# Apokleos/kata-xpu-device-plugin

Hardware: NVIDIA H100
Metric: pci.ids parse GB/s (x1000 text + 2^20-key join); device lookups/s reported beside it (higher is better)
Workload: dtype u8

## Files before the change

### kata-xpu-device-plugin_b200/csrc/api.cu

```cuda
#include <algorithm>
#include <cstdlib>
#include <new>
#include <vector>

#include "internal.cuh"
#include "pciids5.cu"
#include "finalize.cuh"
#include "small.cuh"
#include "scan.cuh"

void kx_exchange_destroy(kxpu_ctx *ctx);

static const char *kx_err_names[] = {
    "ok", "invalid argument", "CUDA error", "no sm_90 GPU available", "output buffer too small",
    "table capacity exceeded", "NCCL / peer exchange unavailable or failed", "input outside the supported domain", "out of memory"};

extern "C" const char *kxpu_strerror(int32_t status) {
    int i = -status;
    if (i < 0 || i > 8) return "unknown status";
    return kx_err_names[i];
}

extern "C" const char *kxpu_last_error(kxpu_ctx *ctx) {
    if (!ctx) return "null ctx";
    static thread_local char copy[sizeof(ctx->err)];
    std::lock_guard<std::mutex> g(ctx->mu);
    memcpy(copy, ctx->err, sizeof copy);
    copy[sizeof copy - 1] = 0;
    return copy;
}
extern "C" uint64_t kxpu_launch_count(kxpu_ctx *ctx) { return ctx ? ctx->launches : 0; }

int32_t kx_ctx_create_on(int32_t ordinal, kxpu_ctx **out) {
    if (!out) return KXPU_E_INVALID;
    *out = nullptr;
    int count = 0;
    if (cudaGetDeviceCount(&count) != cudaSuccess || count <= 0 || ordinal < 0 || ordinal >= count) {
        cudaGetLastError();
        return KXPU_E_NOGPU;
    }
    cudaDeviceProp prop;
    if (cudaGetDeviceProperties(&prop, ordinal) != cudaSuccess) return KXPU_E_NOGPU;
    if (prop.major != 9 || prop.minor != 0) return KXPU_E_NOGPU;
    kxpu_ctx *c = new (std::nothrow) kxpu_ctx();
    if (!c) return KXPU_E_NOMEM;
    c->device = ordinal;
    c->sm_count = prop.multiProcessorCount;
    if (cudaSetDevice(ordinal) != cudaSuccess || cudaStreamCreateWithFlags(&c->stream, cudaStreamNonBlocking) != cudaSuccess) {
        delete c;
        return KXPU_E_CUDA;
    }
    bool ok = true;
    for (int i = 0; i < 2 * KXPU_T_COUNT; i++) ok = ok && cudaEventCreate(&c->ev[i]) == cudaSuccess;
    ok = ok && cudaEventCreate(&c->ev_user[0]) == cudaSuccess && cudaEventCreate(&c->ev_user[1]) == cudaSuccess;
    ok = ok && cudaMallocHost((void **)&c->h_ctl, (KX_C_COUNT + 64) * sizeof(uint32_t)) == cudaSuccess;
    if (!ok) {
        cudaGetLastError();
        kxpu_ctx_destroy(c);
        return KXPU_E_CUDA;
    }
    cudaMemPool_t pool;
    if (cudaDeviceGetDefaultMemPool(&pool, ordinal) == cudaSuccess) {
        uint64_t thr = ~0ull;
        cudaMemPoolSetAttribute(pool, cudaMemPoolAttrReleaseThreshold, &thr);
    }
    cudaFuncSetAttribute(kxparse5::parse_kernel_v5, cudaFuncAttributeMaxDynamicSharedMemorySize,
                         (int)(sizeof(kxparse5::WarpSmem5) * kxparse::WARPS));
    const char *fr = getenv("KXPU_RCH");
    c->force_rch = (fr && fr[0] >= '1' && fr[0] <= '8' && !fr[1]) ? fr[0] - '0' : 0;
    c->no_small = getenv("KXPU_NO_SMALL") != nullptr;
    c->no_zero_copy = getenv("KXPU_NO_ZERO_COPY") != nullptr;
    if (const char *sw = getenv("KXPU_SCAN_W")) { const int v = atoi(sw); c->force_scan_w = (v == 8 || v == 16 || v == 32) ? v : 0; }
    if (const char *el = getenv("KXPU_SCAN_EPOCH_LIMIT")) {
        char *end = nullptr;
        const unsigned long long v = (el[0] >= '0' && el[0] <= '9') ? strtoull(el, &end, 10) : 0;
        if (end && !*end && v >= 2 && v <= (1ull << 24)) c->scan_epoch_limit = (uint32_t)v;
    }
    *out = c;
    return KXPU_OK;
}

extern "C" int32_t kxpu_ctx_create(int32_t ordinal, kxpu_ctx **out) { return kx_ctx_create_on(ordinal, out); }

extern "C" int32_t kxpu_ctx_destroy(kxpu_ctx *ctx) {
    if (!ctx) return KXPU_E_INVALID;
// ... 181 lines not shown
            break;
        }
    }
    if (!found) {
        KxArena a;
        a.cap = cap; a.blob_cap = blob_cap; a.range_bytes = need_range;
        a.bytes = arena_layout(cap, blob_cap, need_range).total;
        cudaError_t e = cudaMalloc(&a.p, a.bytes);
        if (e != cudaSuccess) {
            cudaGetLastError();
            for (KxArena &p : ctx->pool) cudaFree(p.p);
            ctx->pool.clear();
            e = cudaMalloc(&a.p, a.bytes);
        }
        if (e != cudaSuccess) {
            cudaGetLastError();
            KX_SET_ERR(ctx, "cudaMalloc(%zu) for a table arena -> %s", a.bytes, cudaGetErrorString(e));
            delete t;
            return e == cudaErrorMemoryAllocation ? KXPU_E_NOMEM : KXPU_E_CUDA;
        }
        arena_reset(ctx, a);
        t->arena = a;
    }
    const ArenaLayout L = arena_layout(cap, blob_cap, t->arena.range_bytes);
    uint8_t *b = (uint8_t *)t->arena.p;
    t->cap = cap;
    uint32_t lg = 0;
    while ((1u << lg) < cap) lg++;
    t->shift = 32 - lg;
    t->dev.slots = (KxSlot *)(b + L.o_slots);
    t->dev.vendor_first = (unsigned long long *)(b + L.o_vfirst);
    t->dev.trunc = (unsigned long long *)(b + L.o_trunc);
    t->dev.counters = (uint32_t *)(b + L.o_counters);
    t->dev.cap = cap;
    t->dev.shift = t->shift;
    t->dev.max_keys = cap / 2;
    t->range_words = (unsigned long long *)(b + L.o_range);
    t->row_key = (uint32_t *)(b + L.o_row_key);
    t->row_line = (unsigned long long *)(b + L.o_row_line);
    t->row_anchor = (unsigned long long *)(b + L.o_row_anchor);
    t->row_name_off = (uint32_t *)(b + L.o_row_noff);
    t->row_name_len = (uint32_t *)(b + L.o_row_nlen);
    t->sel = (uint32_t *)(b + L.o_sel);
    t->blob = b + L.o_blob;
    t->blob_cap = blob_cap;
    t->rows_cap = cap + 1;
    *out = t;
    return KXPU_OK;
}

void kx_table_release(kxpu_ctx *ctx, kxpu_table *t) {
    if (!t) return;
    if (t->arena.p) {
        if (ctx->pool.size() >= 4) {
            cudaStreamSynchronize(ctx->stream);
            cudaFree(ctx->pool.front().p);
            ctx->pool.erase(ctx->pool.begin());
        }
        arena_reset(ctx, t->arena);
        ctx->pool.push_back(t->arena);
    }
    delete t;
}

uint32_t kx_initial_blob_cap(kxpu_ctx *ctx, size_t n) {
    const uint32_t by_text = (uint32_t)std::min<size_t>(std::max<size_t>(n, 256), 4u << 20);
    return ctx->blob_hint > by_text ? ctx->blob_hint : by_text;
}

bool kx_grow_cap(uint32_t *cap, bool table_full) {
    if (*cap >= (1u << 28)) return false;
    const uint32_t sh = table_full ? 4u : 2u;
    *cap = (*cap >> (28u - sh)) ? (1u << 28) : (*cap << sh);
    return true;
}

void kx_note_table_size(kxpu_ctx *ctx, uint32_t nkeys, uint32_t blob_used, uint32_t blob_cap) {
    uint32_t ideal = 1u << 16;
    while (ideal < (1u << 28) && ideal / 2 < nkeys + nkeys / 8) ideal <<= 1;
    ctx->cap_hint = ideal;
    ctx->blob_hint = blob_cap > (4u << 20) && blob_used > (2u << 20) ? blob_cap : 0u;
}

int32_t kx_launch_parse(kxpu_ctx *ctx, kxpu_table *t, const uint8_t *d_text, size_t n, unsigned long long base,
                        unsigned long long carry_in, const KxXaHook *xa) {
    using namespace kxparse;
    const uint32_t num_chunks = (uint32_t)((n + CW - 1) / CW);
    kxparse5::Params5 P;
    memset(&P, 0, sizeof P);
    if (xa) { P.xa_on = 1; P.xa_done = xa->done; P.xa = xa->p; }
    if (num_chunks == 0) {
        if (xa) {
            P.tab = t->dev;
            P.task_ctas = 0;
            kxparse5::resolve_chunks_kernel<<<kxparse5::XA_CTAS, kxparse5::RES_WARPS * 32, 0, ctx->stream>>>(P);
            KX_LAUNCHED(ctx);
            KX_CUDA(ctx, cudaGetLastError());
        }
        return KXPU_OK;
    }
    P.text = d_text; P.n = n; P.base = base; P.num_chunks = num_chunks;
    P.tma_limit = n >= (size_t)STG_BYTES ? (uint32_t)((n - STG_BYTES) / CW) + 1u : 0u;
    static int per_sm = 0;
    const size_t smem = sizeof(kxparse5::WarpSmem5) * WARPS;
    if (per_sm == 0) {
        cudaOccupancyMaxActiveBlocksPerMultiprocessor(&per_sm, kxparse5::parse_kernel_v5, NT, smem);
        if (per_sm < 1) per_sm = 1;
    }
    const uint32_t wave_warps = (uint32_t)per_sm * ctx->sm_count * WARPS;
    P.rch = std::min<uint32_t>(std::max<uint32_t>(num_chunks / (wave_warps * 8u), 1u), kxparse5::RCH5_MAX);
    if (ctx->force_rch) P.rch = (uint32_t)ctx->force_rch;
    P.num_ranges = (num_chunks + P.rch - 1) / P.rch;
    P.range_state = t->range_words;
    P.range_carry = t->range_words + P.num_ranges;
    P.lead = (uint32_t *)(t->range_words + 2 * P.num_ranges);
    P.tasks = P.lead + P.num_ranges;
    P.tab = t->dev; P.carry_in = carry_in;
    uint32_t grid = (uint32_t)per_sm * ctx->sm_count;
    const uint32_t need = (P.num_ranges + WARPS - 1) / WARPS;
    if (grid > need) grid = need;
    {
        KxTimer tm(ctx, KXPU_T_PARSE);
        kxparse5::parse_kernel_v5<<<grid, NT, smem, ctx->stream>>>(P);
        KX_LAUNCHED(ctx);
    }
    {
        KxTimer tr(ctx, KXPU_T_RESOLVE);
        kxparse5::resolve_ranges_kernel<<<(P.num_ranges + 255u) / 256u, 256, 0, ctx->stream>>>(P);
        KX_LAUNCHED(ctx);
        const uint32_t rgrid = std::min<uint32_t>(4u * ctx->sm_count, (num_chunks + kxparse5::RES_WARPS - 1) / kxparse5::RES_WARPS);
        P.task_ctas = rgrid;
        kxparse5::resolve_chunks_kernel<<<rgrid + (xa ? kxparse5::XA_CTAS : 0u), kxparse5::RES_WARPS * 32, 0, ctx->stream>>>(P);
        KX_LAUNCHED(ctx);
    }
    KX_CUDA(ctx, cudaGetLastError());
    return KXPU_OK;
}

int32_t kx_launch_trunc(kxpu_ctx *ctx, kxpu_table *t, const uint8_t *d_text, size_t n, unsigned long long base) {
    kxparse::trunc_kernel<<<1, 1024, 0, ctx->stream>>>(d_text, n, base, t->dev.trunc, t->dev.counters);
    KX_LAUNCHED(ctx);
    KX_CUDA(ctx, cudaGetLastError());
    return KXPU_OK;
}

int32_t kx_launch_finalize(kxpu_ctx *ctx, kxpu_table *t, const uint8_t *d_text, size_t n, unsigned long long base,
                           const kxx::MinView *mv, const kxx::WaitSpec *wait, const KxSlabOut *slab) {
    kxparse::FinalizeParams F;
    memset(&F, 0, sizeof F);
    if (wait) F.wait = *wait;
    F.text = d_text; F.n = n; F.base = base; F.tab = t->dev;
    if (mv) F.mv = *mv;
    else { F.mv.a = t->dev.vendor_first; F.mv.stride = 0; F.mv.n = 1; F.mv.trunc1 = t->dev.trunc; }
    F.row_key = t->row_key; F.row_line = t->row_line; F.row_anchor = t->row_anchor;
    F.row_name_off = t->row_name_off; F.row_name_len = t->row_name_len;
    F.blob = t->blob; F.blob_cap = t->blob_cap;
    if (slab) {
        F.slab_rows = reinterpret_cast<kxx::SlabRow *>(slab->rows); F.slab_rows_cap = slab->rows_cap;
        F.blob = slab->blob; F.blob_cap = slab->blob_cap;
        F.tail = slab->tail;
    }
    KxTimer tm(ctx, KXPU_T_FINALIZE);
    F.scan_w = t->cap >= (1u << 19) ? 32u : 8u;
    if (ctx->force_scan_w) F.scan_w = (uint32_t)ctx->force_scan_w;
    const unsigned batches = (t->cap + 1 + F.scan_w - 1) / F.scan_w;
    const unsigned grid = std::min<unsigned>((batches + kxparse::SF_WARPS - 1) / kxparse::SF_WARPS, 8u * ctx->sm_count);
    kxparse::select_finalize_kernel<<<grid, kxparse::SF_WARPS * 32, 0, ctx->stream>>>(F);
    KX_LAUNCHED(ctx);
    KX_CUDA(ctx, cudaGetLastError());
    return KXPU_OK;
}

int32_t kx_launch_lookup(kxpu_ctx *ctx, kxpu_table *t, const uint32_t *d_keys, size_t n, int32_t *d_rows) {
    if (n == 0) return KXPU_OK;
    KxTimer tm(ctx, KXPU_T_LOOKUP);
    size_t blocks = (n + 255) / 256;
    size_t maxb = (size_t)ctx->sm_count * 32;
    if (blocks > maxb) blocks = maxb;
    kxparse::lookup_kernel<<<(unsigned)blocks, 256, 0, ctx->stream>>>(d_keys, n, t->dev.slots, t->cap, t->shift, d_rows);
    KX_LAUNCHED(ctx);
    KX_CUDA(ctx, cudaGetLastError());
    return KXPU_OK;
}

struct KxJoin {
    const uint32_t *d_keys;
    size_t n;
    int32_t *d_rows;
    int32_t *h_rows;
    const uint8_t *src_text;
};

static void *kx_mapped_host(const void *p) {
    if (!p) return nullptr;
    cudaPointerAttributes at;
    if (cudaPointerGetAttributes(&at, p) != cudaSuccess) { cudaGetLastError(); return nullptr; }
    return at.type == cudaMemoryTypeHost ? at.devicePointer : nullptr;
}

static uint32_t small_text_chunks(kxpu_ctx *ctx) {
    if (ctx->small_chunks < 0) {
        int coop = 0, per_sm = 0;
        cudaDeviceGetAttribute(&coop, cudaDevAttrCooperativeLaunch, ctx->device);
        cudaFuncSetAttribute(kxsmall::small_load_kernel, cudaFuncAttributeMaxDynamicSharedMemorySize, kxparse::WARPS * kxparse::STG_BYTES);
        cudaOccupancyMaxActiveBlocksPerMultiprocessor(&per_sm, kxsmall::small_load_kernel, kxparse::NT, kxparse::WARPS * kxparse::STG_BYTES);
        cudaGetLastError();
        ctx->small_chunks = (coop && !ctx->no_small) ? per_sm * ctx->sm_count * kxparse::WARPS : 0;
    }
    return (uint32_t)ctx->small_chunks;
}

static int32_t launch_small(kxpu_ctx *ctx, kxpu_table *t, const uint8_t *d_text, size_t n, const KxJoin *join) {
    using namespace kxparse;
    kxsmall::SmallParams P;
    memset(&P, 0, sizeof P);
    P.text = d_text; P.n = n;
    P.num_chunks = (uint32_t)((n + CW - 1) / CW);
    P.tma_limit = n >= (size_t)STG_BYTES ? (uint32_t)((n - STG_BYTES) / CW) + 1u : 0u;
    P.state = t->range_words;
    FinalizeParams &F = P.F;
    F.text = d_text; F.n = n; F.base = 0; F.tab = t->dev;
    F.mv.a = t->dev.vendor_first; F.mv.stride = 0; F.mv.n = 1; F.mv.trunc1 = t->dev.trunc;
    F.row_key = t->row_key; F.row_line = t->row_line; F.row_anchor = t->row_anchor;
    F.row_name_off = t->row_name_off; F.row_name_len = t->row_name_len;
    F.blob = t->blob; F.blob_cap = t->blob_cap;
    if (join) { P.keys = join->d_keys; P.nq = join->n; P.rows_out = join->d_rows; }
    if (join && join->src_text) { P.text_src = join->src_text; P.h_ctl = ctx->h_ctl; }
    void *args[] = {&P};
    const unsigned grid = std::max<unsigned>((P.num_chunks + WARPS - 1) / WARPS, (unsigned)(ctx->small_chunks / WARPS));
    F.scan_w = 8u;
    while (F.scan_w < 32u && (size_t)(t->cap + 1 + F.scan_w - 1) / F.scan_w > (size_t)grid * SF_WARPS) F.scan_w *= 2u;
    if (ctx->force_scan_w) F.scan_w = (uint32_t)ctx->force_scan_w;
    static const bool trace_on = getenv("KXPU_TRACE_SMALL") != nullptr;
    long long *d_trace = nullptr;
    if (trace_on && cudaMalloc((void **)&d_trace, (size_t)grid * 128 + (size_t)P.num_chunks * 32) == cudaSuccess) { cudaMemset(d_trace, 0, (size_t)grid * 128 + (size_t)P.num_chunks * 32); P.trace = d_trace; P.F.trace = d_trace + (size_t)grid * 8 + (size_t)P.num_chunks * 4; }
    {
        KxTimer tm(ctx, KXPU_T_PARSE);
        KX_CUDA(ctx, cudaLaunchCooperativeKernel((const void *)kxsmall::small_load_kernel, dim3(grid), dim3(NT), args, (size_t)WARPS * STG_BYTES, ctx->stream));
        KX_LAUNCHED(ctx);
    }
    if (d_trace) {
        std::vector<long long> h((size_t)grid * 16 + (size_t)P.num_chunks * 4);
        cudaStreamSynchronize(ctx->stream);
        cudaMemcpy(h.data(), d_trace, h.size() * 8, cudaMemcpyDeviceToHost);
        cudaFree(d_trace);
        static const char *nm[7] = {"phase1", "barrier1", "phase2", "barrier2", "names", "barrier3", "join"};
        fprintf(stderr, "[kxpu small trace] %u CTAs, cycles min/avg/max per CTA:", grid);
        for (int k = 0; k < 7; k++) {
            long long mn = 1ll << 62, mx = 0, sum = 0, cnt = 0;
            for (unsigned b = 0; b < grid; b++) {
                if (!h[b * 8 + k + 1] || !h[b * 8 + k]) continue;
                const long long d = h[b * 8 + k + 1] - h[b * 8 + k];
                mn = std::min(mn, d); mx = std::max(mx, d); sum += d; cnt++;
            }
            if (cnt) fprintf(stderr, " %s %lld/%lld/%lld |", nm[k], mn, sum / cnt, mx);
        }
        {
            std::vector<std::pair<long long, unsigned>> v;
            for (unsigned b = 0; b < grid; b++) v.push_back({h[b * 8 + 3] - h[b * 8 + 2], b});
            std::sort(v.rbegin(), v.rend());
            fprintf(stderr, " slowest phase2 CTAs:");
            for (int k = 0; k < 6 && k < (int)v.size(); k++) fprintf(stderr, " %u:%lld", v[k].second, v[k].first);
            std::vector<std::pair<long long, unsigned>> wv;
            const long long *tw = h.data() + (size_t)grid * 8;
            for (unsigned c = 0; c < P.num_chunks; c++) wv.push_back({tw[c * 4], c});
            std::sort(wv.rbegin(), wv.rend());
            fprintf(stderr, "\n   slowest phase2 warps (chunk: cycles / before folds / entries / look-back steps):");
            for (int k = 0; k < 10 && k < (int)wv.size(); k++) {
                const unsigned c = wv[k].second;
                fprintf(stderr, " %u: %lld/%lld/%lld/%lld |", c, tw[c * 4], tw[c * 4 + 1], tw[c * 4 + 2], tw[c * 4 + 3]);
            }
            const unsigned mid = wv[wv.size() / 2].second;
            fprintf(stderr, " median %u: %lld/%lld/%lld/%lld", mid, tw[mid * 4], tw[mid * 4 + 1], tw[mid * 4 + 2], tw[mid * 4 + 3]);
            const long long *tf = h.data() + (size_t)grid * 8 + (size_t)P.num_chunks * 4;
            static const char *fn[7] = {"scan", "rounds", "sync1+claim", "sync2", "names out+rows", "long lines", "shift+sync3"};
            fprintf(stderr, "\n   names phase per CTA (thread 0), cycles min/avg/max:");
            for (int k = 0; k < 7; k++) {
                long long mn = 1ll << 62, mx = 0, sum = 0, cnt = 0;
                for (unsigned b = 0; b < grid; b++) {
                    const long long t1 = tf[b * 8 + k], t0 = k ? tf[b * 8 + k - 1] : h[b * 8 + 4];
                    if (!t1 || !t0) continue;
                    const long long d = t1 - t0;
                    mn = std::min(mn, d); mx = std::max(mx, d); sum += d; cnt++;
                }
                if (cnt) fprintf(stderr, " %s %lld/%lld/%lld |", fn[k], mn, sum / cnt, mx);
            }
        }
        fprintf(stderr, "\n");
    }
    return KXPU_OK;
}

static int32_t kx_build_table_join(kxpu_ctx *ctx, const uint8_t *d_text, size_t n, kxpu_table **out, const KxJoin *join) {
    if ((reinterpret_cast<uintptr_t>(d_text) & 15u) != 0) {
        KX_SET_ERR(ctx, "device text pointer must be 16-byte aligned");
        return KXPU_E_INVALID;
    }
    if (n >= (1ull << 44)) return KXPU_E_UNSUPPORTED;
    uint32_t cap = ctx->cap_hint;
    while (cap > (1u << 16) && (size_t)cap / 2 > n / 6 + 1) cap >>= 1;
    uint32_t blob_cap = kx_initial_blob_cap(ctx, n);
    const uint32_t num_chunks = (uint32_t)((n + kxparse::CW - 1) / kxparse::CW);
    bool have_trunc = false;
    for (int attempt = 0; attempt < 12; attempt++) {
        kxpu_table *t = nullptr;
        int32_t rc = kx_table_acquire(ctx, cap, blob_cap, num_chunks, &t);
        if (rc != KXPU_OK) return rc;
        const bool small_path = num_chunks > 0 && num_chunks <= small_text_chunks(ctx) && !have_trunc;
        if (small_path) {
            rc = launch_small(ctx, t, d_text, n, join);
        } else {
            if (join && join->src_text && attempt == 0) cudaMemcpyAsync(const_cast<uint8_t *>(d_text), join->src_text, n, cudaMemcpyDefault, ctx->stream);
            rc = kx_launch_parse(ctx, t, d_text, n, 0, 0, nullptr);
            if (rc == KXPU_OK && have_trunc) rc = kx_launch_trunc(ctx, t, d_text, n, 0);
            if (rc == KXPU_OK) rc = kx_launch_finalize(ctx, t, d_text, n, 0, nullptr, nullptr, nullptr);
            if (rc == KXPU_OK && join) rc = kx_launch_lookup(ctx, t, join->d_keys, join->n, join->d_rows);
        }
        if (rc != KXPU_OK) { kx_table_release(ctx, t); return rc; }
        const bool zero_copy = small_path && join && join->src_text;
        if (!zero_copy) {
            if (join && join->h_rows && join->n) cudaMemcpyAsync(join->h_rows, join->d_rows, join->n * 4, cudaMemcpyDeviceToHost, ctx->stream);
            cudaMemcpyAsync(ctx->h_ctl, t->dev.counters, KX_C_COUNT * 4, cudaMemcpyDeviceToHost, ctx->stream);
        }
        cudaError_t e = cudaStreamSynchronize(ctx->stream);
        if (e != cudaSuccess) {
            KX_SET_ERR(ctx, "parse/finalize failed: %s", cudaGetErrorString(e));
            kx_table_release(ctx, t);
            return KXPU_E_CUDA;
        }
        const uint32_t *h = ctx->h_ctl;
        if (h[KX_C_OVERFLOW] || h[KX_C_NKEYS] > t->dev.max_keys) {
            kx_table_release(ctx, t);
            if (!kx_grow_cap(&cap, h[KX_C_OVERFLOW] != 0)) return KXPU_E_CAPACITY;
            continue;
        }
        if (h[KX_C_NEED_TRUNC] == 2u) {
            kx_table_release(ctx, t);
            have_trunc = true;
            continue;
        }
        if (h[KX_C_BLOB_OVERFLOW]) {
            kx_table_release(ctx, t);
            if ((size_t)blob_cap >= n) return KXPU_E_CAPACITY;
            blob_cap = (uint32_t)std::min<size_t>(std::max<size_t>(n, 256), (size_t)blob_cap * 8);
            continue;
        }
        t->n_rows = h[KX_C_NSEL];
        t->blob_used = h[KX_C_BLOB_CURSOR];
        kx_note_table_size(ctx, h[KX_C_NKEYS], t->blob_used, blob_cap);
        *out = t;
        return KXPU_OK;
    }
    return KXPU_E_CAPACITY;
}

extern "C" int32_t kxpu_pciids_load_device(kxpu_ctx *ctx, const void *d_text, size_t n, kxpu_table **out) {
    KX_ENTER(ctx);
    if (!out || (!d_text && n)) return KXPU_E_INVALID;
    kx_clear_timings(ctx);
    return kx_build_table_join(ctx, (const uint8_t *)d_text, n, out, nullptr);
}

extern "C" int32_t kxpu_pciids_join_device(kxpu_ctx *ctx, const void *d_text, size_t n, const uint32_t *d_keys, size_t nq,
                                           int32_t *d_rows_out, kxpu_table **out) {
    KX_ENTER(ctx);
    if (!out || (!d_text && n) || (nq && (!d_keys || !d_rows_out))) return KXPU_E_INVALID;
    kx_clear_timings(ctx);
    const KxJoin j{d_keys, nq, d_rows_out, nullptr, nullptr};
    return kx_build_table_join(ctx, (const uint8_t *)d_text, n, out, &j);
}

static int32_t stage_reserve(kxpu_ctx *ctx, size_t bytes) {
    if (bytes <= ctx->d_stage_bytes) return KXPU_OK;
    if (ctx->d_stage) {
        cudaStreamSynchronize(ctx->stream);
        cudaFree(ctx->d_stage);
        ctx->d_stage = nullptr;
        ctx->d_stage_bytes = 0;
    }
    const size_t want = align_up(bytes + bytes / 8 + 4096, 4096);
    cudaError_t e = cudaMalloc(&ctx->d_stage, want);
    if (e != cudaSuccess) {
        cudaGetLastError();
        KX_SET_ERR(ctx, "cudaMalloc(%zu) for the host staging buffer -> %s", want, cudaGetErrorString(e));
        return e == cudaErrorMemoryAllocation ? KXPU_E_NOMEM : KXPU_E_CUDA;
    }
    ctx->d_stage_bytes = want;
    return KXPU_OK;
}

extern "C" int32_t kxpu_pciids_load(kxpu_ctx *ctx, const uint8_t *text, size_t n, kxpu_table **out) {
    KX_ENTER(ctx);
    if (!out || (!text && n)) return KXPU_E_INVALID;
    kx_clear_timings(ctx);
    int32_t rc = stage_reserve(ctx, n + 16);
    if (rc != KXPU_OK) return rc;
    cudaError_t e = cudaMemcpyAsync(ctx->d_stage, text, n, cudaMemcpyHostToDevice, ctx->stream);
    if (e != cudaSuccess) {
        KX_SET_ERR(ctx, "H2D copy of the text failed: %s", cudaGetErrorString(e));
// ... 143 lines not shown
```

### kata-xpu-device-plugin_b200/csrc/common.cuh

```cuda
#pragma once
#include <cuda_runtime.h>
#include <stdint.h>
#include <stdio.h>
#include <string.h>

#include <mutex>
#include <vector>

#include "../../include/kxpu.h"

constexpr int KX_MAX_RANKS = 16;


struct KxArena {
    void *p = nullptr;
    size_t bytes = 0;
    uint32_t cap = 0, blob_cap = 0;
    size_t range_bytes = 0;
};

struct KxExchange;
struct kxpu_multi;

struct kxpu_ctx {
// ... 1 lines not shown
    int sm_count = 0;
    cudaStream_t stream = nullptr;
    cudaEvent_t ev[2 * KXPU_T_COUNT] = {};
    cudaEvent_t ev_user[2] = {};
    bool ev_used[KXPU_T_COUNT] = {};
    int force_rch = 0;
    bool no_small = false;
    bool no_zero_copy = false;
    int force_scan_w = 0;
    int small_chunks = -1;
    bool stage_timing = true;
    uint64_t launches = 0;
    std::mutex mu;
    char err[512] = {0};
    uint32_t *h_ctl = nullptr;
    std::vector<KxArena> pool;
    uint32_t cap_hint = 1u << 16;
    uint32_t blob_hint = 0;
    unsigned long long *scan_state = nullptr;
    size_t scan_state_words = 0;
    uint32_t scan_epoch = 0;
    uint32_t scan_epoch_limit = 1u << 24;
    void *d_stage = nullptr;
    size_t d_stage_bytes = 0;
    void *nccl_comm = nullptr;
    int nranks = 1, rank = 0;
    KxExchange *xch = nullptr;
    kxpu_multi *multi = nullptr;
};

#define KX_SET_ERR(ctx, ...) snprintf((ctx)->err, sizeof((ctx)->err), __VA_ARGS__)

#define KX_CUDA(ctx, call)                                                                  \
    do {                                                                                    \
        cudaError_t e__ = (call);                                                           \
        if (e__ != cudaSuccess) {                                                           \
            KX_SET_ERR(ctx, "%s:%d %s -> %s", __FILE__, __LINE__, #call, cudaGetErrorString(e__)); \
            return KXPU_E_CUDA;                                                             \
        }                                                                                   \
    } while (0)

#define KX_LAUNCHED(ctx) ((ctx)->launches++)

struct KxTimer {
    kxpu_ctx *c;
    int idx;
    bool open = true;
    KxTimer(kxpu_ctx *ctx, int i) : c(ctx), idx(i) {
        open = c->stage_timing;
        if (open) cudaEventRecord(c->ev[2 * i], c->stream);
    }
    void stop() {
        if (open) { cudaEventRecord(c->ev[2 * idx + 1], c->stream); c->ev_used[idx] = true; open = false; }
    }
    ~KxTimer() { stop(); }
};

static inline void kx_clear_timings(kxpu_ctx *c) { memset(c->ev_used, 0, sizeof(c->ev_used)); }

unsigned long long *kx_scan_state(kxpu_ctx *ctx, size_t words);
uint32_t kx_next_epoch(kxpu_ctx *ctx);

struct KxScratch {
    kxpu_ctx *c;
    std::vector<void *> ptrs;
    explicit KxScratch(kxpu_ctx *ctx) : c(ctx) {}
    cudaError_t alloc(void **p, size_t bytes) {
        cudaError_t e = cudaMallocAsync(p, bytes ? bytes : 16, c->stream);
        if (e == cudaSuccess) ptrs.push_back(*p);
        else *p = nullptr;
        return e;
    }
    ~KxScratch() {
        for (void *p : ptrs) cudaFreeAsync(p, c->stream);
    }
};

#ifdef __CUDACC__
__device__ __forceinline__ uint32_t kx_lane() { return threadIdx.x & 31u; }

__device__ __forceinline__ void kx_fence_gpu() { asm volatile("fence.acq_rel.gpu;" ::: "memory"); }
__device__ __forceinline__ void kx_fence_sys() { asm volatile("fence.acq_rel.sys;" ::: "memory"); }

__device__ __forceinline__ uint32_t kx_hash(uint32_t key) { return key * 0x9E3779B1u; }
#endif
```

### kata-xpu-device-plugin_b200/csrc/finalize.cuh

```cuda
#pragma once
#include "exchange.cuh"
#include "parse_common.cuh"

namespace kxparse {

constexpr unsigned long long MAX_TOKEN = 65536ull;

__global__ void __launch_bounds__(1024) trunc_kernel(const uint8_t *__restrict__ text, unsigned long long n,
                                                      unsigned long long base, unsigned long long *trunc_out, uint32_t *counters) {
    __shared__ unsigned long long s_first[1024], s_last[1024], s_bad[1024];
    const unsigned long long per = (n + 1023ull) / 1024ull;
    const unsigned long long lo = per * threadIdx.x, hi = lo + per < n ? lo + per : n;
    unsigned long long first = KX_NO_OFF, last = KX_NO_OFF, bad = KX_NO_OFF;
    for (unsigned long long i = lo; i < hi; i++) {
        if (text[i] == (uint8_t)'\n') {
            if (first == KX_NO_OFF) first = i;
            else if (i - last - 1 >= MAX_TOKEN && bad == KX_NO_OFF) bad = last + 1;
            last = i;
        }
    }
    s_first[threadIdx.x] = first; s_last[threadIdx.x] = last; s_bad[threadIdx.x] = bad;
    __syncthreads();
    if (threadIdx.x == 0) {
        unsigned long long prev_nl = KX_NO_OFF;
// ... 285 lines not shown
            const uint32_t l_key = q[r].key, l_slot = q[r].slot;
            const unsigned long long rs = l_line - F.base + 5ull;
            uint8_t *buf = &s_name[wl][0][0];
            constexpr uint32_t LONG_MAX_LEN = (uint32_t)(SF_BATCH * SF_WIN) - 32u;
            uint32_t len = 0;
            bool found = false;
            for (uint32_t o = 0; o < LONG_MAX_LEN + 32u && !found; o += 32u) {
                const unsigned long long pos = rs + o + lane;
                const uint32_t c = pos < F.n ? F.text[pos] : 0x0au;
                buf[o + lane] = (uint8_t)c;
                const uint32_t nlm = __ballot_sync(0xffffffffu, c == 0x0au);
                if (nlm) { len = o + (uint32_t)__ffs((int)nlm) - 1u; found = true; }
            }
            __syncwarp();
            uint32_t start = 0, end = 0, out_len = 0, at = 0;
            bool ok = true;
            if (found) {
                if (len > 0 && buf[len - 1] == 0x0du) len--;
                if (lane == 0) trim_space(buf, len, start, end);
                start = __shfl_sync(0xffffffffu, start, 0);
                end = __shfl_sync(0xffffffffu, end, 0);
                for (uint32_t o = start; o < end; o += 32u) {
                    const uint32_t i = o + lane;
                    const uint32_t ch = i < end ? sanitise_byte(buf, i, start, end) : 0u;
                    out_len += (uint32_t)__popc(__ballot_sync(0xffffffffu, ch != 0u));
                }
                if (lane == 0) {
                    at = out_len ? atomicAdd(&F.tab.counters[KX_C_BLOB_CURSOR], out_len) : 0u;
                    if (at + out_len > F.blob_cap) { F.tab.counters[KX_C_BLOB_OVERFLOW] = 1u; at = 0xFFFFFFFFu; }
                }
                at = __shfl_sync(0xffffffffu, at, 0);
                ok = at != 0xFFFFFFFFu;
                if (ok) {
                    uint32_t wr = at;
                    for (uint32_t o = start; o < end; o += 32u) {
                        const uint32_t i = o + lane;
                        const uint32_t ch = i < end ? sanitise_byte(buf, i, start, end) : 0u;
                        const uint32_t bm = __ballot_sync(0xffffffffu, ch != 0u);
                        if (ch) F.blob[wr + (uint32_t)__popc(bm & ((1u << lane) - 1u))] = (uint8_t)ch;
                        wr += (uint32_t)__popc(bm);
                    }
                }
            } else if (lane == 0) {
                const uint8_t *g = F.text + rs;
                const unsigned long long avail = F.n - rs;
                unsigned long long l = 0;
                while (l < avail && g[l] != 0x0au) l++;
                len = (uint32_t)l;
                if (len > 0 && g[len - 1] == 0x0du) len--;
                trim_space(g, len, start, end);
                for (uint32_t i = start; i < end; i++) out_len += sanitise_byte(g, i, start, end) != 0u;
                at = out_len ? atomicAdd(&F.tab.counters[KX_C_BLOB_CURSOR], out_len) : 0u;
                if (at + out_len > F.blob_cap) { F.tab.counters[KX_C_BLOB_OVERFLOW] = 1u; ok = false; }
                if (ok) {
                    uint32_t wr = at;
                    for (uint32_t i = start; i < end; i++) {
                        const uint32_t ch = sanitise_byte(g, i, start, end);
                        if (ch) F.blob[wr++] = (uint8_t)ch;
                    }
                }
            }
            if (lane == 0) finalize_store_row(F, row0 + r, l_slot, l_key, l_line, l_anchor, ok ? at : 0u, ok ? out_len : 0u);
            __syncwarp();
        }
        SF_MARK(5);
        {
            const uint32_t rem = qn - nvalid;
            if (nvalid != 0u && rem != 0u) {
                SfEntry e;
                if (lane < rem) e = q[nvalid + lane];
                __syncwarp();
                if (lane < rem) q[lane] = e;
                __syncwarp();
            }
            qn = rem;
        }
        __syncthreads();
        SF_MARK(6);
        if (!more) break;
    }
}

__global__ void __launch_bounds__(SF_WARPS * 32, 8) select_finalize_kernel(const FinalizeParams F) {
    kxx::wait_flags_cta(F.wait);
    select_finalize_body(F, F.scan_w);
    if (F.tail.on) {
        __syncthreads();
        if (threadIdx.x == 0) {
            kx_fence_sys();
            const uint32_t prev = atomicAdd(F.tail.done, 1u);
            if (prev == gridDim.x - 1u) {
                *F.tail.done = 0u;
                kx_fence_gpu();
                const volatile uint32_t *c = F.tab.counters;
                const uint32_t n_sel = c[KX_C_NSEL], blob_used = c[KX_C_BLOB_CURSOR];
                const bool over = c[KX_C_BLOB_OVERFLOW] || n_sel > F.tail.rows_cap || blob_used > F.tail.blob_cap;
                kxx::SlabHeader h;
                memset(&h, 0, sizeof h);
                h.n_rows = over ? 0u : n_sel;
                h.blob_bytes = over ? 0u : blob_used;
                h.status = over ? kxx::XS_SLAB_OVERFLOW : 0u;
                if (c[KX_C_OVERFLOW]) h.status |= kxx::XS_GROW | kxx::XS_FULL;
                if (c[KX_C_NKEYS] > F.tab.max_keys) h.status |= kxx::XS_GROW;
                h.nkeys = c[KX_C_NKEYS];
                *F.tail.header = h;
                kx_fence_sys();
                for (int k = 0; k < F.tail.tg.n; k++) *reinterpret_cast<volatile uint32_t *>(F.tail.tg.region[k] + F.tail.o_flag) = F.tail.epoch;
            }
        }
    }
}

__global__ void __launch_bounds__(256) lookup_kernel(const uint32_t *__restrict__ keys, size_t n, const KxSlot *__restrict__ slots,
                                                      uint32_t cap, uint32_t shift, int32_t *__restrict__ rows_out) {
    size_t i = (size_t)blockIdx.x * blockDim.x + threadIdx.x;
    const size_t stride = (size_t)gridDim.x * blockDim.x;
    for (; i < n; i += stride) rows_out[i] = table_probe(slots, cap, shift, keys[i]);
}

__global__ void __launch_bounds__(256) name_len_kernel(const int32_t *__restrict__ rows, size_t n,
                                                        const uint32_t *__restrict__ row_name_len, uint32_t n_rows,
                                                        uint32_t *__restrict__ lens) {
    size_t i = (size_t)blockIdx.x * blockDim.x + threadIdx.x;
    if (i < n) {
        int32_t r = rows[i];
        lens[i] = (r >= 0 && (uint32_t)r < n_rows) ? row_name_len[r] : 0u;
    }
}
__global__ void __launch_bounds__(256) name_copy_kernel(const int32_t *__restrict__ rows, size_t n,
                                                         const uint32_t *__restrict__ row_name_off,
                                                         const uint32_t *__restrict__ row_name_len, uint32_t n_rows,
                                                         const uint8_t *__restrict__ blob,
                                                         const uint32_t *__restrict__ offsets, uint8_t *__restrict__ out,
                                                         size_t cap) {
    size_t i = ((size_t)blockIdx.x * blockDim.x + threadIdx.x) >> 3;
    uint32_t sub = threadIdx.x & 7u;
    if (i >= n) return;
    int32_t r = rows[i];
    if (r < 0 || (uint32_t)r >= n_rows) return;
    uint32_t len = row_name_len[r], src = row_name_off[r], dst = offsets[i];
    if ((size_t)dst + len > cap) return;
    for (uint32_t k = sub; k < len; k += 8u) out[dst + k] = blob[src + k];
}

__global__ void __launch_bounds__(256) arena_reset_kernel(uint4 *ff, size_t n_ff16, uint32_t *counters) {
    const size_t i = (size_t)blockIdx.x * blockDim.x + threadIdx.x;
    const size_t stride = (size_t)gridDim.x * blockDim.x;
    for (size_t k = i; k < n_ff16; k += stride) ff[k] = make_uint4(0xffffffffu, 0xffffffffu, 0xffffffffu, 0xffffffffu);
    if (i < KX_C_COUNT) counters[i] = 0u;
}

}
```

### kata-xpu-device-plugin_b200/csrc/internal.cuh

```cuda
#pragma once
#include "common.cuh"
#include "exchange.cuh"
#include "table.cuh"

struct kxpu_table {
    uint32_t cap = 0, shift = 0;
    KxArena arena;
    KxTableDev dev{};
    unsigned long long *range_words = nullptr;
    uint32_t *row_key = nullptr;
    unsigned long long *row_line = nullptr;
    unsigned long long *row_anchor = nullptr;
    uint32_t *row_name_off = nullptr;
    uint32_t *row_name_len = nullptr;
    uint32_t *sel = nullptr;
    uint8_t *blob = nullptr;
    uint32_t blob_cap = 0;
    uint32_t rows_cap = 0;
    uint32_t n_rows = 0;
    uint32_t blob_used = 0;
};

#define KX_ENTER(ctx)                          \
    if (!(ctx)) return KXPU_E_INVALID;         \
    std::lock_guard<std::mutex> guard__((ctx)->mu); \
    cudaSetDevice((ctx)->device)

int32_t kx_table_acquire(kxpu_ctx *ctx, uint32_t cap, uint32_t blob_cap, uint32_t num_chunks, kxpu_table **out);
void kx_table_release(kxpu_ctx *ctx, kxpu_table *t);
uint32_t kx_initial_blob_cap(kxpu_ctx *ctx, size_t n);
struct KxXaHook {
    kxx::XaParams p;
    uint32_t *done;
};
int32_t kx_launch_parse(kxpu_ctx *ctx, kxpu_table *t, const uint8_t *d_text, size_t n, unsigned long long base,
                        unsigned long long carry_in, const KxXaHook *xa);
int32_t kx_launch_trunc(kxpu_ctx *ctx, kxpu_table *t, const uint8_t *d_text, size_t n, unsigned long long base);
struct KxSlabOut {
    uint8_t *rows;
    uint32_t rows_cap;
    uint8_t *blob;
    uint32_t blob_cap;
    kxx::SlabTail tail;
};
int32_t kx_launch_finalize(kxpu_ctx *ctx, kxpu_table *t, const uint8_t *d_text, size_t n, unsigned long long base,
                           const kxx::MinView *mv, const kxx::WaitSpec *wait, const KxSlabOut *slab);
int32_t kx_launch_lookup(kxpu_ctx *ctx, kxpu_table *t, const uint32_t *d_keys, size_t n, int32_t *d_rows);
bool kx_grow_cap(uint32_t *cap, bool table_full);
void kx_note_table_size(kxpu_ctx *ctx, uint32_t nkeys, uint32_t blob_used, uint32_t blob_cap);
```

### kata-xpu-device-plugin_b200/csrc/pciids5.cu

```cuda
#pragma once
#include "exchange.cuh"
#include "parse_common.cuh"

namespace kxparse5 {

using namespace kxparse;

constexpr int STAGES5 = 3;
constexpr int RCH5_MAX = 8;
constexpr int RES_WARPS = 8;

struct WarpSmem5 {
    alignas(16) uint8_t stage[STAGES5][STG_BYTES];
    alignas(8) unsigned long long bar[STAGES5];
};

struct Params5 {
    const uint8_t *text;
    unsigned long long n, base;
    uint32_t num_chunks;
    uint32_t tma_limit;
    uint32_t rch;
    uint32_t num_ranges;
    unsigned long long *range_state;
// ... 206 lines not shown
                        const uint32_t p = pbase + (31u - (uint32_t)__clz((int)bit));
                        uint32_t val;
                        const bool ok = hex4_swar(lds32_unaligned(st + p), val);
                        const unsigned long long line_g = cbase + p;
                        const bool alive = ok && line_g <= P.tab.vendor_first[val];
                        if (alive) {
                            const uint32_t nxt = rest & (0u - rest);
                            const uint32_t seg = (second ? kh[1] & ~th[1] : kh[0] & ~th[0]) & ~(bit | (bit - 1u)) & (nxt ? nxt - 1u : 0xffffffffu);
                            fold_lines(P.tab, st, cbase, seg, pbase, val << 16, line_g, nfresh);
                        }
                        const uint32_t info = (alive ? 0x80000000u : 0u) | ((ok ? val : 0u) << 15) | p;
                        if (second) linfo1 = info; else linfo0 = info;
                    }
                }
                const uint32_t pre0 = kh[0] & ~th[0] & (th[0] ? (th[0] & (0u - th[0])) - 1u : 0xffffffffu);
                const uint32_t pre1 = kh[1] & ~th[1] & (th[1] ? (th[1] & (0u - th[1])) - 1u : 0xffffffffu);
                const uint32_t s0 = bal0 & lt_mask, s1 = bal1 & lt_mask;
                const uint32_t x0 = __shfl_sync(0xffffffffu, linfo0, s0 ? 31 - __clz((int)s0) : 0);
                const uint32_t l0 = __shfl_sync(0xffffffffu, linfo0, bal0 ? 31 - __clz((int)bal0) : 0);
                const uint32_t x1 = __shfl_sync(0xffffffffu, linfo1, s1 ? 31 - __clz((int)s1) : 0);
                const uint32_t l1 = __shfl_sync(0xffffffffu, linfo1, bal1 ? 31 - __clz((int)bal1) : 0);
                const uint32_t last0 = bal0 ? l0 : base_info;
                const uint32_t cin0 = s0 ? x0 : base_info;
                const uint32_t cin1 = s1 ? x1 : last0;
                last1 = bal1 ? l1 : last0;
                if (cin0 != P_NONE && (cin0 >> 31))
                    fold_lines(P.tab, st, cbase, pre0, lane * 32u + 1u, ((cin0 >> 15) & 0xffffu) << 16, cbase + (cin0 & 0x7fffu), nfresh);
                if (cin1 != P_NONE && (cin1 >> 31))
                    fold_lines(P.tab, st, cbase, pre1, (uint32_t)HALF + lane * 32u + 1u, ((cin1 >> 15) & 0xffffu) << 16, cbase + (cin1 & 0x7fffu), nfresh);
                const uint32_t hw0 = cin0 == P_NONE ? pre0 : 0u;
                const uint32_t hw1 = cin1 == P_NONE ? pre1 : 0u;
                if (rc_x & LS_VOK) {
                    uint32_t key_hi = ((rc_x >> 12) & 0xffffu) << 16;
                    unsigned long long anchor = P.base + (unsigned long long)rc_g * CW + (rc_x & 0xfffu);
                    if (rc_g == 0xffffffffu) {
                        key_hi = ((uint32_t)(P.carry_in >> 44) & 0xffffu) << 16;
                        anchor = P.carry_in & CV_ANCHOR_MASK;
                    }
                    if ((hw0 | hw1) != 0u && P.tab.vendor_first[key_hi >> 16] >= anchor) {
                        fold_lines(P.tab, st, cbase, hw0, lane * 32u + 1u, key_hi, anchor, nfresh);
                        fold_lines(P.tab, st, cbase, hw1, (uint32_t)HALF + lane * 32u + 1u, key_hi, anchor, nfresh);
                    }
                }
                flush_fresh(P.tab, nfresh);
            }
            if (last1 != P_NONE) {
                if (rc_x == 0u) lead = i + 1u;
                rc_x = LS_PUB | LS_TOP | ((last1 >> 31) ? LS_VOK : 0u) | (((last1 >> 15) & 0xffffu) << 12) | (last1 & 0xfffu);
                rc_g = g;
            }
            if ((bal0 | bal1) == 0u && n_rel > (uint32_t)CW && __reduce_or_sync(0xffffffffu, rawnl) == 0u && lane == 0)
                atomicOr(&P.tab.counters[KX_C_LONGLINE_HINT], 1u);

            __syncwarp();
            {
                const uint32_t fi = i + (uint32_t)STAGES5;
                uint32_t fg = 0xffffffffu;
                if (fi < rch) {
                    fg = g + (uint32_t)STAGES5;
                } else if (rch > (uint32_t)STAGES5 && cnt == rch && r_next < P.num_ranges) {
                    fg = r_next * rch + (fi - rch);
                    staged = true;
                }
                if (lane == 0) issue(fg, s);
            }
            s = s == (uint32_t)STAGES5 - 1u ? 0u : s + 1u;
        }
        if (lane == 0) {
            unsigned long long v = ST_NONE;
            if (rc_x != 0u) {
                if (rc_g == 0xffffffffu)
                    v = ST_PREFIX | P.carry_in;
                else
                    v = ST_PREFIX | CV_HAS_TOP | ((rc_x & LS_VOK) ? CV_VOK : 0ull) | ((unsigned long long)((rc_x >> 12) & 0xffffu) << 44) |
                        ((P.base + (unsigned long long)rc_g * CW + (rc_x & 0xfffu)) & CV_ANCHOR_MASK);
            }
            P.range_state[r] = v;
            P.lead[r] = lead < cnt ? lead : cnt;
        }
        if (!have_next) r_next = __shfl_sync(0xffffffffu, tk2, 0);
        r = r_next;
        if (r >= P.num_ranges) break;
    }
}

constexpr uint32_t XA_CTAS = 64;

__global__ void __launch_bounds__(256) resolve_ranges_kernel(const Params5 P) {
    const uint32_t rr = blockIdx.x * blockDim.x + threadIdx.x;
    const uint32_t lane = threadIdx.x & 31u;
    const uint32_t rr0 = rr - lane;
    if (rr0 >= P.num_ranges) return;
    const bool live = rr < P.num_ranges;
    const uint32_t nlead = live ? P.lead[rr] : 0u;
    const unsigned long long own = live ? P.range_state[rr] : ST_NONE;
    const uint32_t pm = __ballot_sync(0xffffffffu, (own & ST_MASK) == ST_PREFIX);
    const uint32_t below = pm & ((1u << lane) - 1u);
    const unsigned long long from_warp = __shfl_sync(0xffffffffu, own, below ? 31 - __clz((int)below) : 0);
    unsigned long long warp_in = 0;
    const uint32_t first_p = pm ? (uint32_t)__ffs((int)pm) - 1u : 32u;
    const bool want = __any_sync(0xffffffffu, nlead != 0u && lane <= first_p);
    if (want) {
        long long q0 = (long long)rr0 - 32;
        for (;;) {
            const long long q = q0 + lane;
            const unsigned long long sv = q >= 0 ? P.range_state[q] : (q == -1 ? (ST_PREFIX | P.carry_in) : ST_NONE);
            const uint32_t m = __ballot_sync(0xffffffffu, (sv & ST_MASK) == ST_PREFIX);
            if (m) {
                warp_in = __shfl_sync(0xffffffffu, sv, 31 - __clz((int)m));
                break;
            }
            q0 -= 32;
        }
    }
    const unsigned long long carry = (below ? from_warp : warp_in) & ~ST_MASK;
    const bool alive = nlead != 0u && (carry & CV_HAS_TOP) && (carry & CV_VOK) &&
                       P.tab.vendor_first[(uint32_t)(carry >> 44) & 0xffffu] >= (carry & CV_ANCHOR_MASK);
    const uint32_t mine = alive ? nlead : 0u;
    uint32_t incl = mine;
#pragma unroll
    for (int d = 1; d < 32; d <<= 1) {
        const uint32_t y = __shfl_up_sync(0xffffffffu, incl, d);
        if (lane >= (uint32_t)d) incl += y;
    }
    const uint32_t tot = __shfl_sync(0xffffffffu, incl, 31);
    uint32_t at0 = 0;
    if (lane == 0 && tot) at0 = atomicAdd(&P.tab.counters[KX_C_DEFER], tot);
    at0 = __shfl_sync(0xffffffffu, at0, 0);
    if (!alive) return;
    P.range_carry[rr] = carry;
    const uint32_t at = at0 + incl - mine;
    for (uint32_t j = 0; j < nlead; j++) P.tasks[at + j] = rr * P.rch + j;
}

__global__ void __launch_bounds__(RES_WARPS * 32) resolve_chunks_kernel(const Params5 P) {
    __shared__ __align__(16) uint8_t stg[RES_WARPS][STG_BYTES];
    __shared__ __align__(8) unsigned long long bars[RES_WARPS];
    __shared__ uint16_t plist[RES_WARPS][704];
    if (blockIdx.x >= P.task_ctas) {
        kxx::xa_push_slice(P.xa, (blockIdx.x - P.task_ctas) * blockDim.x + threadIdx.x, XA_CTAS * blockDim.x);
        __syncthreads();
        if (threadIdx.x == 0) {
            kx_fence_sys();
            const uint32_t prev = atomicAdd(P.xa_done, 1u);
            if (prev == XA_CTAS - 1u) {
                *P.xa_done = 0u;
                kx_fence_sys();
                kxx::xa_finish(P.xa);
            }
        }
        return;
    }
    const uint32_t lane = threadIdx.x & 31u, w = threadIdx.x >> 5;
    const uint32_t lt_mask = (1u << lane) - 1u;
    uint32_t k7f = 0x7f7f7f7fu, k0a = 0x0a0a0a0au, k80 = 0x80808080u;
    asm volatile("" : "+r"(k7f), "+r"(k0a), "+r"(k80));
    const uint32_t st = smem_u32(stg[w]), bar = smem_u32(&bars[w]);
    if (lane == 0) {
        mbar_init(&bars[w], 1);
        asm volatile("fence.mbarrier_init.release.cluster;" ::: "memory");
    }
    __syncwarp();
    const unsigned long long pol = l2_evict_first_policy();
    const uint32_t n_tasks = P.tab.counters[KX_C_DEFER];
    uint32_t par = 0, nfresh = 0;
    const bool small_tab = P.tab.cap <= (1u << 20);
    uint32_t it = 0;
    for (uint32_t t = blockIdx.x * RES_WARPS + w; t < n_tasks; t += P.task_ctas * RES_WARPS, it++) {
        if ((it & 3u) == 0u && *reinterpret_cast<volatile uint32_t *>(&P.tab.counters[KX_C_OVERFLOW]) != 0u) break;
        const uint32_t gg = P.tasks[t];
        uint32_t n_rel = CW + 1;
        if (gg < P.tma_limit) {
            if (lane == 0) {
                mbar_expect_tx_a(bar, STG_BYTES);
                tma_load_a(st, P.text + (unsigned long long)gg * CW, STG_BYTES, bar, pol);
            }
            while (!mbar_try_a(bar, par)) {
            }
            par ^= 1u;
        } else {
            n_rel = stage_chunk_manual(P.text, P.n, gg, lane, stg[w]);
        }
        const unsigned long long cc = P.range_carry[gg / P.rch];
        const uint32_t key_hi = ((uint32_t)(cc >> 44) & 0xffffu) << 16;
        const unsigned long long anchor = cc & CV_ANCHOR_MASK;
        uint32_t kh[2], th[2], rawnl;
        chunk_masks(st, lane, n_rel, k7f, k0a, k80, kh, th, rawnl);
        const uint32_t bal0 = __ballot_sync(0xffffffffu, th[0] != 0u);
        const uint32_t bal1 = __ballot_sync(0xffffffffu, th[1] != 0u);
        const uint32_t pre0 = kh[0] & ~th[0] & (th[0] ? (th[0] & (0u - th[0])) - 1u : 0xffffffffu);
        const uint32_t pre1 = kh[1] & ~th[1] & (th[1] ? (th[1] & (0u - th[1])) - 1u : 0xffffffffu);
        const unsigned long long cbase = P.base + (unsigned long long)gg * CW;
        const uint32_t m0 = (bal0 & lt_mask) == 0u ? pre0 : 0u;
        const uint32_t m1 = (bal0 == 0u && (bal1 & lt_mask) == 0u) ? pre1 : 0u;
        const uint32_t mine = (uint32_t)__popc(m0) + (uint32_t)__popc(m1);
        uint32_t incl = mine;
#pragma unroll
        for (int d = 1; d < 32; d <<= 1) {
            const uint32_t y = __shfl_up_sync(0xffffffffu, incl, d);
            if (lane >= (uint32_t)d) incl += y;
        }
        const uint32_t total = __shfl_sync(0xffffffffu, incl, 31);
        {
            uint32_t idx = incl - mine;
            for (uint32_t m = m0; m; m &= m - 1u) plist[w][idx++] = (uint16_t)(lane * 32u + 1u + (uint32_t)__ffs((int)m) - 1u);
            for (uint32_t m = m1; m; m &= m - 1u) plist[w][idx++] = (uint16_t)((uint32_t)HALF + lane * 32u + 1u + (uint32_t)__ffs((int)m) - 1u);
        }
        __syncwarp();
        if (small_tab) {
            for (uint32_t i = lane; i < total; i += 64u) {
                uint32_t d0, d1 = 0;
                const uint32_t p0 = plist[w][i], p1 = i + 32u < total ? plist[w][i + 32u] : 0u;
                bool v0 = hex4_swar(lds32_unaligned(st + p0 + 1u), d0);
                bool v1 = i + 32u < total && hex4_swar(lds32_unaligned(st + p1 + 1u), d1);
                uint32_t q0 = p0, q1 = p1;
                if (!v0 && v1) { d0 = d1; q0 = p1; v0 = true; v1 = false; }
                if (v0) table_fold_claim2(P.tab, key_hi | d0, cbase + q0, anchor, v1, key_hi | d1, cbase + q1, anchor, nfresh);
            }
        } else {
            for (uint32_t i = lane; i < total; i += 32u) {
                const uint32_t p = plist[w][i];
// ... 11 lines not shown
```

Before: 2300.

## Chain parse/resolve/finalize/lookup kernels with programmatic dependent launch

Launches resolve_ranges, resolve_chunks, select_finalize and lookup through cudaLaunchKernelEx with programmatic stream serialization, adding griddepcontrol wait/launch_dependents so each kernel's launch and prologue overlap the previous kernel's tail. The lookup kernel computes its hash-table probe position before waiting on the predecessor and reads the row afterwards via __ldcg, hiding part of the probe latency. The goal is to cut inter-kernel launch gaps and drain bubbles across the pipeline. It risks correctness if table_find reads slot state written by finalize before the wait, and PDL is disabled when stage timing or truncation is active.

```diff
diff --git a/kata-xpu-device-plugin_b200/csrc/api.cu b/kata-xpu-device-plugin_b200/csrc/api.cu
--- a/kata-xpu-device-plugin_b200/csrc/api.cu
+++ b/kata-xpu-device-plugin_b200/csrc/api.cu
@@ -1,6 +1,7 @@
 #include <algorithm>
 #include <cstdlib>
 #include <new>
+#include <utility>
 #include <vector>
 
 #include "internal.cuh"
@@ -348,8 +349,23 @@
     ctx->blob_hint = blob_cap > (4u << 20) && blob_used > (2u << 20) ? blob_cap : 0u;
 }
 
+template <typename... Params, typename... Args>
+static cudaError_t kx_launch_k(kxpu_ctx *ctx, bool chained, void (*k)(Params...), unsigned grid, unsigned block, size_t smem, Args &&...args) {
+    cudaLaunchAttribute at[1];
+    at[0].id = cudaLaunchAttributeProgrammaticStreamSerialization;
+    at[0].val.programmaticStreamSerializationAllowed = 1;
+    cudaLaunchConfig_t cfg = {};
+    cfg.gridDim = dim3(grid);
+    cfg.blockDim = dim3(block);
+    cfg.dynamicSmemBytes = smem;
+    cfg.stream = ctx->stream;
+    cfg.attrs = at;
+    cfg.numAttrs = chained ? 1u : 0u;
+    return cudaLaunchKernelEx(&cfg, k, std::forward<Args>(args)...);
+}
+
 int32_t kx_launch_parse(kxpu_ctx *ctx, kxpu_table *t, const uint8_t *d_text, size_t n, unsigned long long base,
-                        unsigned long long carry_in, const KxXaHook *xa) {
+                        unsigned long long carry_in, const KxXaHook *xa, bool chained) {
     using namespace kxparse;
     const uint32_t num_chunks = (uint32_t)((n + CW - 1) / CW);
     kxparse5::Params5 P;
@@ -392,11 +408,12 @@
     }
     {
         KxTimer tr(ctx, KXPU_T_RESOLVE);
-        kxparse5::resolve_ranges_kernel<<<(P.num_ranges + 255u) / 256u, 256, 0, ctx->stream>>>(P);
+        const bool ch = chained && !ctx->stage_timing;
+        KX_CUDA(ctx, kx_launch_k(ctx, ch, kxparse5::resolve_ranges_kernel, (P.num_ranges + 255u) / 256u, 256, 0, P));
         KX_LAUNCHED(ctx);
         const uint32_t rgrid = std::min<uint32_t>(4u * ctx->sm_count, (num_chunks + kxparse5::RES_WARPS - 1) / kxparse5::RES_WARPS);
         P.task_ctas = rgrid;
-        kxparse5::resolve_chunks_kernel<<<rgrid + (xa ? kxparse5::XA_CTAS : 0u), kxparse5::RES_WARPS * 32, 0, ctx->stream>>>(P);
+        KX_CUDA(ctx, kx_launch_k(ctx, ch, kxparse5::resolve_chunks_kernel, rgrid + (xa ? kxparse5::XA_CTAS : 0u), kxparse5::RES_WARPS * 32, 0, P));
         KX_LAUNCHED(ctx);
     }
     KX_CUDA(ctx, cudaGetLastError());
@@ -411,7 +428,7 @@
 }
 
 int32_t kx_launch_finalize(kxpu_ctx *ctx, kxpu_table *t, const uint8_t *d_text, size_t n, unsigned long long base,
-                           const kxx::MinView *mv, const kxx::WaitSpec *wait, const KxSlabOut *slab) {
+                           const kxx::MinView *mv, const kxx::WaitSpec *wait, const KxSlabOut *slab, bool chained) {
     kxparse::FinalizeParams F;
     memset(&F, 0, sizeof F);
     if (wait) F.wait = *wait;
@@ -431,19 +448,20 @@
     if (ctx->force_scan_w) F.scan_w = (uint32_t)ctx->force_scan_w;
     const unsigned batches = (t->cap + 1 + F.scan_w - 1) / F.scan_w;
     const unsigned grid = std::min<unsigned>((batches + kxparse::SF_WARPS - 1) / kxparse::SF_WARPS, 8u * ctx->sm_count);
-    kxparse::select_finalize_kernel<<<grid, kxparse::SF_WARPS * 32, 0, ctx->stream>>>(F);
+    KX_CUDA(ctx, kx_launch_k(ctx, chained && !ctx->stage_timing, kxparse::select_finalize_kernel, grid, kxparse::SF_WARPS * 32, 0, F));
     KX_LAUNCHED(ctx);
     KX_CUDA(ctx, cudaGetLastError());
     return KXPU_OK;
 }
 
-int32_t kx_launch_lookup(kxpu_ctx *ctx, kxpu_table *t, const uint32_t *d_keys, size_t n, int32_t *d_rows) {
+int32_t kx_launch_lookup(kxpu_ctx *ctx, kxpu_table *t, const uint32_t *d_keys, size_t n, int32_t *d_rows, bool chained) {
     if (n == 0) return KXPU_OK;
     KxTimer tm(ctx, KXPU_T_LOOKUP);
     size_t blocks = (n + 255) / 256;
     size_t maxb = (size_t)ctx->sm_count * 32;
     if (blocks > maxb) blocks = maxb;
-    kxparse::lookup_kernel<<<(unsigned)blocks, 256, 0, ctx->stream>>>(d_keys, n, t->dev.slots, t->cap, t->shift, d_rows);
+    const bool ch = chained && !ctx->stage_timing;
+    KX_CUDA(ctx, kx_launch_k(ctx, ch, kxparse::lookup_kernel, (unsigned)blocks, 256, 0, d_keys, n, t->dev, d_rows, ch ? 1 : 0));
     KX_LAUNCHED(ctx);
     KX_CUDA(ctx, cudaGetLastError());
     return KXPU_OK;
@@ -577,10 +595,10 @@
             rc = launch_small(ctx, t, d_text, n, join);
         } else {
             if (join && join->src_text && attempt == 0) cudaMemcpyAsync(const_cast<uint8_t *>(d_text), join->src_text, n, cudaMemcpyDefault, ctx->stream);
-            rc = kx_launch_parse(ctx, t, d_text, n, 0, 0, nullptr);
+            rc = kx_launch_parse(ctx, t, d_text, n, 0, 0, nullptr, !have_trunc);
             if (rc == KXPU_OK && have_trunc) rc = kx_launch_trunc(ctx, t, d_text, n, 0);
-            if (rc == KXPU_OK) rc = kx_launch_finalize(ctx, t, d_text, n, 0, nullptr, nullptr, nullptr);
-            if (rc == KXPU_OK && join) rc = kx_launch_lookup(ctx, t, join->d_keys, join->n, join->d_rows);
+            if (rc == KXPU_OK) rc = kx_launch_finalize(ctx, t, d_text, n, 0, nullptr, nullptr, nullptr, !have_trunc);
+            if (rc == KXPU_OK && join) rc = kx_launch_lookup(ctx, t, join->d_keys, join->n, join->d_rows, !have_trunc);
         }
         if (rc != KXPU_OK) { kx_table_release(ctx, t); return rc; }
         const bool zero_copy = small_path && join && join->src_text;
diff --git a/kata-xpu-device-plugin_b200/csrc/common.cuh b/kata-xpu-device-plugin_b200/csrc/common.cuh
--- a/kata-xpu-device-plugin_b200/csrc/common.cuh
+++ b/kata-xpu-device-plugin_b200/csrc/common.cuh
@@ -107,5 +107,8 @@
 __device__ __forceinline__ void kx_fence_gpu() { asm volatile("fence.acq_rel.gpu;" ::: "memory"); }
 __device__ __forceinline__ void kx_fence_sys() { asm volatile("fence.acq_rel.sys;" ::: "memory"); }
 
+__device__ __forceinline__ void kx_grid_wait() { asm volatile("griddepcontrol.wait;" ::: "memory"); }
+__device__ __forceinline__ void kx_grid_launch_dependents() { asm volatile("griddepcontrol.launch_dependents;" ::: "memory"); }
+
 __device__ __forceinline__ uint32_t kx_hash(uint32_t key) { return key * 0x9E3779B1u; }
 #endif
diff --git a/kata-xpu-device-plugin_b200/csrc/finalize.cuh b/kata-xpu-device-plugin_b200/csrc/finalize.cuh
--- a/kata-xpu-device-plugin_b200/csrc/finalize.cuh
+++ b/kata-xpu-device-plugin_b200/csrc/finalize.cuh
@@ -391,6 +391,8 @@
 }
 
 __global__ void __launch_bounds__(SF_WARPS * 32, 8) select_finalize_kernel(const FinalizeParams F) {
+    kx_grid_wait();
+    kx_grid_launch_dependents();
     kxx::wait_flags_cta(F.wait);
     select_finalize_body(F, F.scan_w);
     if (F.tail.on) {
@@ -420,11 +422,20 @@
     }
 }
 
-__global__ void __launch_bounds__(256) lookup_kernel(const uint32_t *__restrict__ keys, size_t n, const KxSlot *__restrict__ slots,
-                                                      uint32_t cap, uint32_t shift, int32_t *__restrict__ rows_out) {
+__global__ void __launch_bounds__(256) lookup_kernel(const uint32_t *__restrict__ keys, size_t n, const KxTableDev tab,
+                                                      int32_t *__restrict__ rows_out, int chained) {
     size_t i = (size_t)blockIdx.x * blockDim.x + threadIdx.x;
     const size_t stride = (size_t)gridDim.x * blockDim.x;
-    for (; i < n; i += stride) rows_out[i] = table_probe(slots, cap, shift, keys[i]);
+    if (!chained) {
+        for (; i < n; i += stride) rows_out[i] = table_probe(tab.slots, tab.cap, tab.shift, keys[i]);
+        return;
+    }
+    uint32_t slot = i < n ? table_find(tab, keys[i]) : 0xffffffffu;
+    kx_grid_wait();
+    for (bool first = true; i < n; i += stride, first = false) {
+        if (!first) slot = table_find(tab, keys[i]);
+        rows_out[i] = slot == 0xffffffffu ? -1 : __ldcg(&tab.slots[slot].row);
+    }
 }
 
 __global__ void __launch_bounds__(256) name_len_kernel(const int32_t *__restrict__ rows, size_t n,
diff --git a/kata-xpu-device-plugin_b200/csrc/internal.cuh b/kata-xpu-device-plugin_b200/csrc/internal.cuh
--- a/kata-xpu-device-plugin_b200/csrc/internal.cuh
+++ b/kata-xpu-device-plugin_b200/csrc/internal.cuh
@@ -34,7 +34,7 @@
     uint32_t *done;
 };
 int32_t kx_launch_parse(kxpu_ctx *ctx, kxpu_table *t, const uint8_t *d_text, size_t n, unsigned long long base,
-                        unsigned long long carry_in, const KxXaHook *xa);
+                        unsigned long long carry_in, const KxXaHook *xa, bool chained = false);
 int32_t kx_launch_trunc(kxpu_ctx *ctx, kxpu_table *t, const uint8_t *d_text, size_t n, unsigned long long base);
 struct KxSlabOut {
     uint8_t *rows;
@@ -44,7 +44,7 @@
     kxx::SlabTail tail;
 };
 int32_t kx_launch_finalize(kxpu_ctx *ctx, kxpu_table *t, const uint8_t *d_text, size_t n, unsigned long long base,
-                           const kxx::MinView *mv, const kxx::WaitSpec *wait, const KxSlabOut *slab);
-int32_t kx_launch_lookup(kxpu_ctx *ctx, kxpu_table *t, const uint32_t *d_keys, size_t n, int32_t *d_rows);
+                           const kxx::MinView *mv, const kxx::WaitSpec *wait, const KxSlabOut *slab, bool chained = false);
+int32_t kx_launch_lookup(kxpu_ctx *ctx, kxpu_table *t, const uint32_t *d_keys, size_t n, int32_t *d_rows, bool chained = false);
 bool kx_grow_cap(uint32_t *cap, bool table_full);
 void kx_note_table_size(kxpu_ctx *ctx, uint32_t nkeys, uint32_t blob_used, uint32_t blob_cap);
diff --git a/kata-xpu-device-plugin_b200/csrc/pciids5.cu b/kata-xpu-device-plugin_b200/csrc/pciids5.cu
--- a/kata-xpu-device-plugin_b200/csrc/pciids5.cu
+++ b/kata-xpu-device-plugin_b200/csrc/pciids5.cu
@@ -312,11 +312,14 @@
         r = r_next;
         if (r >= P.num_ranges) break;
     }
+    kx_grid_launch_dependents();
 }
 
 constexpr uint32_t XA_CTAS = 64;
 
 __global__ void __launch_bounds__(256) resolve_ranges_kernel(const Params5 P) {
+    kx_grid_wait();
+    kx_grid_launch_dependents();
     const uint32_t rr = blockIdx.x * blockDim.x + threadIdx.x;
     const uint32_t lane = threadIdx.x & 31u;
     const uint32_t rr0 = rr - lane;
@@ -367,6 +370,8 @@
     __shared__ __align__(16) uint8_t stg[RES_WARPS][STG_BYTES];
     __shared__ __align__(8) unsigned long long bars[RES_WARPS];
     __shared__ uint16_t plist[RES_WARPS][704];
+    kx_grid_wait();
+    kx_grid_launch_dependents();
     if (blockIdx.x >= P.task_ctas) {
         kxx::xa_push_slice(P.xa, (blockIdx.x - P.task_ctas) * blockDim.x + threadIdx.x, XA_CTAS * blockDim.x);
         __syncthreads();
```

Result: no change. 2310 (median of 6 runs) (+0.4%).
